# jliu/graph-normalizing-flows

Measured on AMD Instinct MI355X. Metric: node-updates/sec (fwd+logdet) on community_medium batch, higher is better.
Workload: dtype f32; 1 GPU; config2: community_medium batch=64/GPU (64 graphs total), 8-step GRevNet fwd+logdet, D=64 L=256 K=5 avg_then_mlp eps=1 leaky_relu(0.2), sparse topology+self loops; nodes_total=2718, edges_total=32202, nodes_rank0=2718, edges_rank0=32202, weights=N(0,2/(fan_in+fan_out)), seed 99, last layer x0.25, parallelism=single GPU

## Files before the change

graph-normalizing-flows_amd/csrc/gnf_fused.hip:

```cpp
#include <cstring>
#include "gnf_common.h"

namespace gnf {

static constexpr int kFusedThreads = 512;
static constexpr int kLdsLimit = 160 * 1024;
static constexpr int kRowptrPad = 40;
static constexpr int kColCap = 2048;

static inline int pad16(int v) { return (v + 15) & ~15; }

int64_t packed_floats(const GnfMlp* m) {
    int64_t tot = 0;
    for (int j = 0; j < m->num_layers; ++j) {
        const int64_t ip = pad16(m->dims[j]), op = pad16(m->dims[j + 1]);
        tot += 2 * ip * op + op;
    }
    return tot;
}

__global__ __launch_bounds__(256) void k_pack_layer(const float* __restrict__ W,
                                                    const float* __restrict__ b, int I, int O, int Ip,
                                                    int Op, float* __restrict__ wout,
                                                    float* __restrict__ bout, float* __restrict__ wtout) {
    const int64_t nw = (int64_t)Ip * Op;
    const int64_t i = (int64_t)blockIdx.x * 256 + threadIdx.x;
    if (i < nw) {
        const int q = (int)(i & 3);
        const int lane = (int)((i >> 2) & 63);
        const int64_t blk = i >> 8;
        const int kgs = Ip >> 4;
        const int nts = Op >> 4;
        const int kg = (int)(blk / nts), nt = (int)(blk % nts);
        (void)kgs;
        const int k = 16 * kg + 4 * (lane >> 4) + q;
        const int c = 16 * nt + (lane & 15);
        wout[i] = (k < I && c < O) ? W[(int64_t)k * O + c] : 0.f;
        const int nts_t = Ip >> 4;
        const int kg_t = (int)(blk / nts_t), nt_t = (int)(blk % nts_t);
        const int ko = 16 * kg_t + 4 * (lane >> 4) + q;
        const int ci = 16 * nt_t + (lane & 15);
        wtout[i] = (ci < I && ko < O) ? W[(int64_t)ci * O + ko] : 0.f;
    } else if (i < nw + Op) {
        const int c = (int)(i - nw);
        bout[c] = c < O ? b[c] : 0.f;
    }
}

static int64_t packed_weight_floats(const GnfMlp* m) {
    int64_t tot = 0;
    for (int j = 0; j < m->num_layers; ++j) tot += (int64_t)pad16(m->dims[j]) * pad16(m->dims[j + 1]);
    return tot;
}

int launch_pack_mlp(const GnfMlp* m, float* packed, hipStream_t st) {
    int64_t woff = 0, boff = packed_weight_floats(m);
    int64_t toff = boff;
    for (int j = 0; j < m->num_layers; ++j) toff += pad16(m->dims[j + 1]);
    for (int j = 0; j < m->num_layers; ++j) {
        const int I = m->dims[j], O = m->dims[j + 1], Ip = pad16(I), Op = pad16(O);
        const int64_t tot = (int64_t)Ip * Op + Op;
        hipLaunchKernelGGL(k_pack_layer, dim3((unsigned)((tot + 255) / 256)), dim3(256), 0, st, m->W[j],
                           m->b[j], I, O, Ip, Op, packed + woff, packed + boff, packed + toff + woff);
        GNF_LAUNCH_CHECK("k_pack_layer");
        woff += (int64_t)Ip * Op;
        boff += Op;
    }
    return GNF_OK;
}


}
#include "gnf_fused_dev.h"
#include "gnf_attn_front_dev.h"
namespace gnf {

#ifdef GNF_TRACE
static constexpr int kTraceSlots = 32, kTraceCoupled = kTraceSlots - 2, kTraceEnd = kTraceSlots - 1;
static constexpr int kTracePhFlushed = 20;
__shared__ unsigned long long s_trace[kFusedThreads / 64][kTraceSlots];
static unsigned long long* g_trace_buf = nullptr;
static int g_trace_cap = 0, g_trace_next = 0;
extern "C" __attribute__((visibility("default"))) void gnf_trace_set_buffer(unsigned long long* buf, int cap) {
    g_trace_buf = buf, g_trace_cap = cap, g_trace_next = 0;
}
__device__ __forceinline__ void geo_stamp(int slot) {
    __builtin_amdgcn_sched_barrier(0);
    const unsigned long long t = __builtin_readcyclecounter();
    if ((threadIdx.x & 63) == 0) s_trace[threadIdx.x >> 6][slot] = t;
    __builtin_amdgcn_sched_barrier(0);
}
__device__ __forceinline__ void geo_stamp_after(int slot, float landed) {
    asm volatile("" ::"v"(landed));
    geo_stamp(slot);
}
#define GNF_STAMP(SLOT) geo_stamp(SLOT)
#define GNF_STAMP_AFTER(SLOT, V) geo_stamp_after(SLOT, V)
#else
#define GNF_STAMP(SLOT) ((void)0)
#define GNF_STAMP_AFTER(SLOT, V) ((void)0)
#endif

template <class Mv>
__device__ __forceinline__ double add_moved(double v, Mv&& mv) {
    const int lo = mv(__double2loint(v)), hi = mv(__double2hiint(v));
    return v + __hiloint2double(hi, lo);
}
__device__ __forceinline__ double wave_sum_lane0(double v) {
    v = add_moved(v, [](int x) { return (int)__builtin_amdgcn_permlane32_swap((unsigned)x, (unsigned)x, false, false)[1]; });
    v = add_moved(v, [](int x) { return (int)__builtin_amdgcn_permlane16_swap((unsigned)x, (unsigned)x, false, false)[1]; });
    v = add_moved(v, [](int x) { return __builtin_amdgcn_update_dpp(0, x, 0x108, 0xf, 0xf, true); });
    v = add_moved(v, [](int x) { return __builtin_amdgcn_update_dpp(0, x, 0x104, 0xf, 0xf, true); });
    v = add_moved(v, [](int x) { return __builtin_amdgcn_update_dpp(0, x, 0x102, 0xf, 0xf, true); });
    v = add_moved(v, [](int x) { return __builtin_amdgcn_update_dpp(0, x, 0x101, 0xf, 0xf, true); });
    return v;
}

struct CoupleOwn {
    float xu = 0.f;
    float* dst = nullptr;
    double* part = nullptr;
    double* sq_part = nullptr;
    int inverse = 0;
};
template <int TM, bool STASH, bool FRONT, bool ROWLD, bool PLAIN, class Args, class FArgs, class RArgs>
__device__ __forceinline__ void couple_tile(const Args& a, const FArgs& fa, const RArgs& rla, const int H, const int LS, float* s_lds,
                                            const float* t_lds, float* xn_lds, const float* bn_lds, double* red, int tile, int row0,
                                            int tid, int wave, int lane, [[maybe_unused]] const CoupleOwn& own = CoupleOwn{}) {
    [[maybe_unused]] auto bn_part = [&]() -> double* {
        if constexpr (PLAIN) return nullptr; else return a.bn_part;
    };
    double local = 0.0, local2 = 0.0;
    for (int idx = tid; idx < TM * H; idx += kFusedThreads) {
        const int rl = idx / H, f = idx - rl * H;
        const int r = row0 + rl;
        if (bn_part()) xn_lds[rl * LS + f] = 0.f;
        bool live;
        if constexpr (PLAIN) live = own.dst != nullptr; else live = r < a.n_nodes;
        if (live) {
            float sv = s_lds[rl * LS + f], tv = t_lds[rl * LS + f];
            [[maybe_unused]] const int HPb = (H + 15) & ~15;
            if constexpr (!PLAIN) {
                if (a.residual) {
                    float xr = a.x_cond[(int64_t)r * a.ld + f];
                    if constexpr (FRONT) {
                        if (fa.bn_part) xr = xr * bn_lds[f] + bn_lds[HPb + f];
                    }
                    sv += xr;
                    tv += xr;
                }
            }
            float xv;
            if constexpr (PLAIN) xv = own.xu; else xv = a.x_upd_src[(int64_t)r * a.ld + f];
            if constexpr (FRONT) {
                if (a.bnu_const) xv = xv * bn_lds[2 * HPb + f] + bn_lds[3 * HPb + f];
                else if (a.bnu_inv[0]) xv = (xv - bn_lds[f]) / bn_lds[HPb + f] * bn_lds[2 * HPb + f] + bn_lds[3 * HPb + f];
            }
            int inverse;
            if constexpr (PLAIN) inverse = own.inverse; else inverse = a.inverse;
            const float xn = inverse ? (xv - tv) * expf(-sv) : xv * expf(sv) + tv;
            if constexpr (PLAIN) *own.dst = xn; else a.x_upd[(int64_t)r * a.ld + f] = xn;
            local += (double)sv;
            local2 += (double)xn * (double)xn;
            if constexpr (ROWLD) s_lds[rl * LS + f] = sv;
            if (bn_part()) xn_lds[rl * LS + f] = xn;
            if constexpr (STASH) {
                a.stash_st[0][(int64_t)r * H + f] = sv;
                a.stash_st[1][(int64_t)r * H + f] = tv;
            }
        }
    }
    if constexpr (PLAIN) GNF_STAMP(kTraceCoupled);
    if constexpr (PLAIN) {
        constexpr int NW = kFusedThreads / 64;
        const bool sq = own.sq_part != nullptr;
        local = wave_sum_lane0(local);
        if (sq) local2 = wave_sum_lane0(local2);
        if (lane == 0) {
            red[wave] = local;
            if (sq) red[NW + wave] = local2;
        }
        __syncthreads();
        if (tid == 0) {
            double tot = 0.0 + local;
            for (int w = 1; w < NW; ++w) tot += red[w];
            *own.part = tot;
            if (sq) {
                double tot2 = 0.0 + local2;
                for (int w = 1; w < NW; ++w) tot2 += red[NW + w];
                *own.sq_part = tot2;
            }
        }
        return;
    }
    for (int off = 32; off > 0; off >>= 1) local += __shfl_down(local, off, 64);
    if (lane == 0) red[wave] = local;
    __syncthreads();
    if (tid == 0) {
        double tot = 0.0;
        for (int w = 0; w < kFusedThreads / 64; ++w) tot += red[w];
        a.partials[tile] = tot;
    }
    if constexpr (!PLAIN) {
        if (a.bn_part) {
            __syncthreads();
            for (int i = tid; i < 2 * H; i += kFusedThreads) {
                const int f = i >> 1, which = i & 1;
                double acc = 0.0;
                for (int rl = 0; rl < TM; ++rl) {
                    const double v = (double)xn_lds[rl * LS + f];
                    acc += which ? v * v : v;
                }
                a.bn_part[((int64_t)tile * H + f) * 2 + which] = acc;
            }
        }
    }
    if (a.sq_partials) {
        for (int off = 32; off > 0; off >>= 1) local2 += __shfl_down(local2, off, 64);
        __syncthreads();
        if (lane == 0) red[wave] = local2;
        __syncthreads();
        if (tid == 0) {
            double tot = 0.0;
            for (int w = 0; w < kFusedThreads / 64; ++w) tot += red[w];
            a.sq_partials[tile] = tot;
        }
    }
    if constexpr (ROWLD) {
        __syncthreads();
        constexpr int TPR = kFusedThreads / TM;
        const int rl = tid / TPR, l = tid % TPR;
        double acc = 0.0;
        for (int f = l; f < H; f += TPR) acc += (double)s_lds[rl * LS + f];
        for (int off = TPR / 2; off > 0; off >>= 1) acc += __shfl_down(acc, off, TPR);
        if (l == 0 && row0 + rl < a.n_nodes) rla.row[row0 + rl] = acc;
    }
}

__device__ __forceinline__ int nets2_tile(int bid, int nwg) {
    const int xcd = bid & 7, qd = nwg >> 3, rm = nwg & 7;
    return (xcd < rm ? xcd * (qd + 1) : rm * (qd + 1) + (xcd - rm) * qd) + (bid >> 3);
}

template <int MT, int NETS, bool STASH = false, bool FRONT = false, bool FIXED = false, bool ROWLD = false>
__global__ __launch_bounds__(kFusedThreads) void k_half_fused(const FusedArgs a, const FrontArgs fa, const RowLdArgs rla) {
    extern __shared__ __attribute__((aligned(16))) float smem[];
    static_assert(!FRONT || (MT == 1 && NETS == 2), "the attention prologue exists for the 16-row both-nets shape");
    static_assert(!ROWLD || (NETS == 2 && !STASH), "per-row log-det: the both-nets inference instances (one net per workgroup couples in k_coupling)");
    constexpr int TM = 16 * MT;
    constexpr int WPN = 8 / NETS;
    const int LS = a.LS;
    auto buf = [&](int net_, int pp_) -> float* { return smem + (2 * net_ + pp_) * TM * LS; };
    int base_floats = 2 * NETS * TM * LS;
    if constexpr (FRONT) {
// ... 182 lines not shown
        const bool v4 = (a.in0 & 3) == 0 && ((reinterpret_cast<uintptr_t>(a.h0[net0]) | reinterpret_cast<uintptr_t>(a.h0[NETS == 2 ? 1 : net0])) & 15) == 0;
        if (v4) {
            const int q4 = in0p >> 2;
            for (int idx = tid; idx < TM * q4; idx += kFusedThreads) {
                const int rl = idx / q4, c = (idx - rl * q4) * 4;
                const int r = row0 + rl;
                const bool live = r < a.n_nodes && c < a.in0;
                const f32x4 z4 = {0.f, 0.f, 0.f, 0.f};
                const f32x4 v0 = live ? *reinterpret_cast<const f32x4*>(a.h0[net0] + (int64_t)r * a.in0 + c) : z4;
                f32x4 v1 = z4;
                if (NETS == 2 && live) v1 = *reinterpret_cast<const f32x4*>(a.h0[1] + (int64_t)r * a.in0 + c);
                *reinterpret_cast<f32x4*>(buf(0, 0) + rl * LS + c) = v0;
                if (NETS == 2) *reinterpret_cast<f32x4*>(buf(1, 0) + rl * LS + c) = v1;
            }
        } else
        for (int idx = tid; idx < TM * in0p; idx += kFusedThreads) {
            const int rl = idx / in0p, c = idx - rl * in0p;
            const int r = row0 + rl;
            const bool live = r < a.n_nodes && c < a.in0;
            buf(0, 0)[rl * LS + c] = live ? a.h0[net0][(int64_t)r * a.in0 + c] : 0.f;
            if (NETS == 2) buf(1, 0)[rl * LS + c] = live ? a.h0[1][(int64_t)r * a.in0 + c] : 0.f;
        }
    } else {
        const TileAgg ta{a.col, a.x_cond, a.ld, a.n_nodes, row0, H, a.in0, a.ipg[0] * 16, a.mean, a.concat, a.eps, a.cond_copy};
        tile_aggregate<TM, kFusedThreads, kColCap>(ta, s_rowptr, s_col, buf(0, 0), NETS == 2 ? buf(1, 0) : nullptr, LS,
                                                   STASH ? a.stash_h0 : nullptr, tid);
    }
    __syncthreads();
    }

    int pp = 0;
    for (int j = 0; j < a.K; ++j) {
        const float* in_lds = buf(nl, pp);
        float* out_lds = buf(nl, pp ^ 1);
        const float slope = (j == a.K - 1) ? 1.f : (a.act == GNF_ACT_RELU ? 0.f : a.alpha);
        while (cur.layer == j) {
            const WChunk c = cur;
            const WChunk nxt = next_chunk(c);
            const WChunk nx = nxt.layer < a.K ? nxt : c;
            const float* bl = bias_lds + nl * a.bias_tot + c.boff;
            constexpr bool kThin = MT == 1;
            const bool thin_ok = kThin && thin_for(j), thin_nx = kThin && thin_for(nx.layer);
            constexpr int EPI = STASH ? EPI_EX : EPI_PLAIN;
            EpiArgs ea{};
            if constexpr (STASH) {
                ea.mode = 0;
                ea.mask = j < a.K - 1 ? fmask + (size_t)(nl * (a.K - 1) + j) * (MT * 4) * a.stash_mld : nullptr;
                ea.mld = a.stash_mld;
            }
            if (c.nv >= 4)
                mlp_chunk<MT, 4, EPI>(in_lds, LS, c, nx, WPN, bl, out_lds, slope, lane, b_pre, ea, thin_nx);
            else if (c.nv == 3)
                mlp_chunk<MT, 3, EPI>(in_lds, LS, c, nx, WPN, bl, out_lds, slope, lane, b_pre, ea, thin_nx);
            else if (c.nv == 2)
                mlp_chunk<MT, 2, EPI>(in_lds, LS, c, nx, WPN, bl, out_lds, slope, lane, b_pre, ea, thin_nx);
            else if (kThin && thin_ok && chunk_is_thin(c))
                mlp_chunk_thin(in_lds, LS, c, nx, WPN, bl, out_lds, slope, lane, b_pre);
            else
                mlp_chunk<MT, 1, EPI>(in_lds, LS, c, nx, WPN, bl, out_lds, slope, lane, b_pre, ea, thin_nx);
            cur = nxt;
        }
        if constexpr (STASH && NETS == 2) {
            if (j >= 1) {
#pragma unroll
                for (int q = 0; q < 2; ++q)
                    tile_dump<TM, kFusedThreads, true>(buf(q, pp), LS, a.stash_act[q][j], (int64_t)a.stash_ld, a.stash_w[j - 1], row0,
                                                       a.n_nodes, tid);
            }
        }
        pp ^= 1;
        __syncthreads();
    }

    if constexpr (STASH) {
        const int total_words = 2 * (a.K - 1) * (MT * 4) * a.stash_mld;
        unsigned long long* gm = a.stash_mask + (size_t)tile * total_words;
        for (int i = tid; i < total_words; i += kFusedThreads) gm[i] = fmask[i];
    }
    if (NETS == 1) {
        const float* o_lds = buf(0, pp);
        float* dst = a.st_out[net0];
        for (int idx = tid; idx < TM * H; idx += kFusedThreads) {
            const int rl = idx / H, f = idx - rl * H;
            const int r = row0 + rl;
            if (r < a.n_nodes)
                dst[(int64_t)r * H + f] = o_lds[rl * LS + f] + (a.residual ? a.x_cond[(int64_t)r * a.ld + f] : 0.f);
        }
    } else {
        couple_tile<TM, STASH, FRONT, ROWLD, false>(a, fa, rla, H, LS, buf(0, pp), buf(1, pp), buf(0, pp ^ 1), bn_lds, red, tile, row0, tid,
                                                    wave, lane);
    }
}


struct GeoArgs {
    const int32_t* rowptr;
    const int32_t* col;
    const float* x_cond;
    float* x_upd;
    const float* x_upd_src;
    float* cond_copy;
    double* partials;
    double* sq_partials;
    const float* wp[2];
    int64_t ld;
    int32_t n_nodes, n_tiles;
    float eps, alpha;
    int32_t mean, act, inverse;
#ifdef GNF_TRACE
    unsigned long long* trace;
#endif
};

template <class T>
__device__ __forceinline__ T hold_v(T v) {
    asm volatile("" : "+v"(v));
    return v;
}
template <class T>
__device__ __forceinline__ T* hold_v(T* p) {
    asm volatile("" : "+v"(p));
    return (T*)(__attribute__((address_space(1))) T*)p;
}

template <int IN0G, int LG, int K, int HG>
struct GeoLayout {
    static constexpr int kWpn = 4;
    static constexpr int kFragFloats = 64 * 4;
    static_assert(kFragFloats * sizeof(float) == 1024 && sizeof(f32x4) == 16, "GNF_LOAD_B addresses 1 KiB fragment blocks, 16 bytes per lane");
    static_assert(K >= 2 && IN0G >= 1 && IN0G == HG, "combine = agg: the layer-0 input is as wide as the half that is rewritten");
    static_assert(LG == 4 * kWpn, "a wave owns exactly four column tiles of a hidden layer: one mlp_chunk<1, 4> per layer");
    static_assert(HG <= kWpn && LG <= kThinStages, "the output layer is at most one thin chunk per wave");
    static constexpr int ipg(int j) { return j == 0 ? IN0G : LG; }
    static constexpr int ont(int j) { return j == K - 1 ? HG : LG; }
    static constexpr int woff(int j) { return j == 0 ? 0 : woff(j - 1) + ipg(j - 1) * ont(j - 1) * kFragFloats; }
    static constexpr int boff(int j) { return j == 0 ? 0 : boff(j - 1) + 16 * ont(j - 1); }
    static constexpr int kBias = woff(K);
    static constexpr int kLS = 16 * (LG > IN0G ? LG : IN0G) + 4;
    static constexpr int kRed = 2 * (kFusedThreads / 64);
    static constexpr int kBiasBlock = boff(K);
    static constexpr size_t kBiasAt = (size_t)2 * 2 * 16 * kLS * sizeof(float) + kRed * sizeof(double) + (kRowptrPad + kColCap) * sizeof(int);
    static constexpr size_t kLds = kBiasAt + (size_t)2 * kBiasBlock * sizeof(float);
    static_assert(kBiasAt % 16 == 0 && kBiasBlock % 4 == 0, "the bias block is written and read in 16-byte pieces");
    static_assert(2 * (kBiasBlock / 4) <= 2 * kFusedThreads && 2 * (kBiasBlock / 4) - kFusedThreads <= 16,
                  "one 16-byte piece per thread, and a second one for at most 16 threads");
    static_assert(kLds > (size_t)kLdsLimit / 2, "one workgroup per CU");
    static_assert(woff(1) == 16 * IN0G * 16 * LG && kBias == 16 * IN0G * 16 * LG + (K - 2) * 256 * LG * LG + 16 * LG * 16 * HG,
                  "sum of Ip x Op over the layers");
    static_assert(kLds <= (size_t)kLdsLimit, "activation buffers in LDS");
    static_assert(LG == 2 * kPhaseTs && kPhaseTs == kFusedThreads / 64, "a wave owns exactly two column tiles of a hidden layer of EACH net: one mlp_phase per net and layer");
    static_assert(2 * HG <= kWpn, "the output layer's 2 HG accumulator chains go to waves 0 .. 2 HG - 1: one per SIMD");
};

template <int IN0G, int LG, int K, int HG, bool PHASES = false>
__global__ __launch_bounds__(kFusedThreads) void k_half_fused_geo(const GeoArgs a) {
    extern __shared__ __attribute__((aligned(16))) float smem[];
    using G = GeoLayout<IN0G, LG, K, HG>;
    constexpr int TM = 16, WPN = G::kWpn, LS = G::kLS, H = 16 * HG, IN0 = 16 * IN0G;
    static_assert(TM * H == kFusedThreads && IN0 == H, "one own-row element per thread, the same one in the gather and in the coupling");
    GNF_STAMP(0);
    auto buf = [&](int net_, int pp_) -> float* { return smem + (2 * net_ + pp_) * TM * LS; };
    double* red = reinterpret_cast<double*>(smem + 2 * 2 * TM * LS);
    int* s_rowptr = reinterpret_cast<int*>(red + G::kRed);
    int* s_col = s_rowptr + kRowptrPad;
    [[maybe_unused]] float* s_bias = smem + G::kBiasAt / sizeof(float);

    const int tid = threadIdx.x;
    const int wave = __builtin_amdgcn_readfirstlane(tid >> 6), lane = tid & 63;
    const int nl = wave / WPN;
    const int wl = (wave % WPN + nl * (WPN / 2)) % WPN;
    const int voff = lane * 16;

    const float* wnet = a.wp[PHASES ? 0 : nl];
    [[maybe_unused]] const float* wnet1 = a.wp[1];
    [[maybe_unused]] const int wt_own = (wave + kPhaseTs - HG) % kPhaseTs;
    if constexpr (PHASES) asm volatile("" ::"s"(wnet1));
#ifdef GNF_TRACE
    asm volatile("" ::"s"(a.trace));
#endif
    asm volatile("" ::"s"(a.rowptr), "s"(a.col), "s"(a.x_cond), "s"(a.x_upd), "s"(a.x_upd_src), "s"(a.cond_copy), "s"(a.partials),
                 "s"(a.sq_partials), "s"(wnet), "s"(a.ld), "s"(a.n_nodes), "s"(a.n_tiles), "s"(a.eps), "s"(a.alpha), "s"(a.mean), "s"(a.act),
                 "s"(a.inverse));
    const int tile = nets2_tile(blockIdx.x, a.n_tiles);
    const int row0 = tile * TM;

    const int rp_row = row0 + (lane < TM ? lane : TM);
    const int rp_reg = a.rowptr[rp_row < a.n_nodes ? rp_row : a.n_nodes];
    CoupleOwn own;
    float xc_own;
    {
        const int r = row0 + tid / H, f = tid % H;
        const bool live = r < a.n_nodes;
        const int64_t at = (int64_t)(live ? r : a.n_nodes - 1) * a.ld + f;
        xc_own = a.x_cond[at];
        own.xu = a.x_upd_src[at];
        own.dst = hold_v(live ? a.x_upd + at : nullptr);
        own.part = hold_v(a.partials + tile);
        own.sq_part = hold_v(a.sq_partials ? a.sq_partials + tile : nullptr);
        own.inverse = hold_v(a.inverse);
    }
    [[maybe_unused]] constexpr int NPC = G::kBiasBlock / 4;
    [[maybe_unused]] f32x4 bias_pc, bias_pc2;
    [[maybe_unused]] const int bias_at2 = kFusedThreads + (lane & 15);
    static_assert(kFusedThreads >= NPC && kFusedThreads + 15 < 2 * NPC, "pieces past kFusedThreads are the second net's");
    if constexpr (PHASES) {
        bias_pc = *reinterpret_cast<const f32x4*>((tid < NPC ? wnet : wnet1) + G::kBias + 4 * (tid < NPC ? tid : tid - NPC));
        bias_pc2 = *reinterpret_cast<const f32x4*>(wnet1 + G::kBias + 4 * (bias_at2 - NPC));
    }
    __builtin_amdgcn_sched_barrier(0);

    auto chunk = [&](auto jc) -> WChunk {
        constexpr int j = decltype(jc)::value;
        WChunk c;
        c.wbase = wnet + G::woff(j);
        c.wbytes = (unsigned)G::ipg(j) * (unsigned)G::ont(j) * 1024u;
        c.ipg = G::ipg(j);
        c.ont = G::ont(j);
        c.boff = G::boff(j);
        c.nt0 = wl;
        c.nv = j == K - 1 ? 1 : 4;
        c.layer = j;
        return c;
    };
    const bool last_mine = wl < HG;

    if (tid <= TM) s_rowptr[tid] = rp_reg;
    const int seg_beg = __builtin_amdgcn_readlane(rp_reg, 0);
    const int seg_len = __builtin_amdgcn_readlane(rp_reg, TM) - seg_beg;
    GNF_STAMP(1);

    const bool staged = seg_len <= kColCap;
    int col_reg = 0;
    if (staged && tid < seg_len) col_reg = a.col[seg_beg + tid];
    __builtin_amdgcn_sched_barrier(0);
    f32x4 b_pre[kPF][4];
    [[maybe_unused]] f32x4 ph_b_pre[kPhasePF][2];
    [[maybe_unused]] auto ph_pf = [](int j) constexpr { return G::ipg(j) < kPhasePF ? G::ipg(j) : kPhasePF; };
    [[maybe_unused]] f32x4 ph_bias[2][K - 1][2];
    [[maybe_unused]] const int thin_net = wave >= HG && wave < 2 * HG;
    [[maybe_unused]] const bool thin_mine = wave < 2 * HG;
    [[maybe_unused]] const int thin_tile = thin_mine ? (thin_net ? wt_own : wave) : 0;
    BiasRegs<4> bias_h[K - 1];
    BiasRegs<1> bias_o;
    if constexpr (PHASES) {
        const __amdgpu_buffer_rsrc_t rs0 =
            __builtin_amdgcn_make_buffer_rsrc(const_cast<float*>(wnet), 0, G::ipg(0) * G::ont(0) * 1024, 0x00020000);
#pragma unroll
        for (int u = 0; u < ph_pf(0); ++u)
#pragma unroll
            for (int b = 0; b < 2; ++b) ph_b_pre[u][b] = GNF_LOAD_B(rs0, voff, (u * G::ont(0) + wave + kPhaseTs * b) * 1024);
    } else {
    prefetch_chunk(chunk(std::integral_constant<int, 0>{}), WPN, voff, b_pre, true);
    const float* bnet = wnet + G::kBias + 16 * wl + (lane & 15);
#pragma unroll
    for (int j = 0; j < K - 1; ++j)
#pragma unroll
        for (int b = 0; b < 4; ++b) bias_h[j].v[b] = bnet[G::boff(j) + 16 * WPN * b];
    bias_o.v[0] = bnet[G::boff(K - 1) - (last_mine ? 0 : 16 * wl)];
    }
    __builtin_amdgcn_sched_barrier(0);
    if constexpr (PHASES) {
        *reinterpret_cast<f32x4*>(s_bias + 4 * tid) = bias_pc;
        if (tid < 2 * NPC - kFusedThreads) *reinterpret_cast<f32x4*>(s_bias + 4 * bias_at2) = bias_pc2;
    }
    if (staged) {
        if (tid < seg_len) s_col[tid] = col_reg;
        for (int i = tid + kFusedThreads; i < seg_len; i += kFusedThreads) s_col[i] = a.col[seg_beg + i];
    }
    __syncthreads();
    GNF_STAMP(2);
    if constexpr (PHASES) {
        __builtin_amdgcn_sched_barrier(0);
#pragma unroll
        for (int q = 0; q < 2; ++q) {
            const float* bq = s_bias + q * G::kBiasBlock + 16 * (q ? wt_own : wave) + 4 * (lane >> 4);
#pragma unroll
            for (int j = 0; j < K - 1; ++j)
#pragma unroll
                for (int b = 0; b < 2; ++b) ph_bias[q][j][b] = *reinterpret_cast<const f32x4*>(bq + G::boff(j) + 16 * kPhaseTs * b);
        }
        bias_o.v[0] = s_bias[thin_net * G::kBiasBlock + G::boff(K - 1) + 16 * thin_tile + (lane & 15)];
    }
    const TileAgg ta{a.col, a.x_cond, a.ld, a.n_nodes, row0, H, IN0, IN0, a.mean, 0, a.eps, a.cond_copy};
    tile_gather<TM, kFusedThreads, kColCap>(ta, s_rowptr, s_col, buf(0, 0), buf(1, 0), LS, nullptr, tid, OwnRow{xc_own});
    __syncthreads();
    GNF_STAMP(3);

    const float slope_h = a.act == GNF_ACT_RELU ? 0.f : a.alpha;
    if constexpr (PHASES) {
        const int lrow = lane & 15, lgrp = lane >> 4;
        const int lane_at = lrow * LS + 4 * lgrp;
        f32x4 acc_s[2], acc_t[2], a_pre[kPhasePF];
#pragma unroll
        for (int u = 0; u < ph_pf(0); ++u) a_pre[u] = *reinterpret_cast<const f32x4*>(buf(0, 0) + lane_at + 16 * u);
        WChunk thin;
        thin.wbase = (thin_net ? wnet1 : wnet) + G::woff(K - 1);
        thin.wbytes = (unsigned)G::ipg(K - 1) * (unsigned)G::ont(K - 1) * 1024u;
        thin.ipg = G::ipg(K - 1), thin.ont = G::ont(K - 1), thin.boff = G::boff(K - 1), thin.nt0 = thin_tile, thin.nv = 1, thin.layer = K - 1;
        epi_static_for<K - 1>([&](auto jc) {
            constexpr int j = decltype(jc)::value;
            constexpr int pj = j & 1;
#pragma unroll
            for (int b = 0; b < 2; ++b) acc_s[b] = ph_bias[0][j][b];
            GNF_STAMP(4 + 4 * j);
            mlp_phase<G::ipg(j), G::ont(j), ph_pf(j), (j > 0), PH_NEXT_HIDDEN, G::ipg(j), G::ont(j), ph_pf(j)>(
                buf(0, pj) + lane_at, wnet + G::woff(j), wave, acc_s, a_pre, ph_b_pre, acc_t, buf(1, pj) + lane_at + 16 * wt_own, slope_h,
                buf(1, pj) + lane_at, wnet1 + G::woff(j), wt_own, thin, b_pre, voff, [&] { GNF_STAMP(5 + 4 * j); });
#pragma unroll
            for (int b = 0; b < 2; ++b) acc_t[b] = ph_bias[1][j][b];
            GNF_STAMP(6 + 4 * j);
            constexpr int jn = j + 1 < K - 1 ? j + 1 : j;
            mlp_phase<G::ipg(j), G::ont(j), ph_pf(j), true, (j + 1 < K - 1 ? PH_NEXT_HIDDEN : PH_NEXT_THIN), G::ipg(jn), G::ont(jn), ph_pf(jn)>(
                buf(1, pj) + lane_at, wnet1 + G::woff(j), wt_own, acc_t, a_pre, ph_b_pre, acc_s, buf(0, pj ^ 1) + lane_at + 16 * wave, slope_h,
                buf(0, pj ^ 1) + lane_at, wnet + G::woff(jn), wave, thin, b_pre, voff, [&] { GNF_STAMP(7 + 4 * j); });
        });
        constexpr int po = (K - 1) & 1;
        phase_flush(acc_t, buf(1, po) + lane_at + 16 * wt_own, slope_h);
        GNF_STAMP(kTracePhFlushed);
        phase_barrier();
        GNF_STAMP(kTracePhFlushed + 1);
        if (thin_mine) mlp_chunk_thin(buf(thin_net, po), LS, thin, thin, kPhaseTs, bias_o, buf(thin_net, po ^ 1), 1.f, lane, b_pre);
        __syncthreads();
        GNF_STAMP(kTracePhFlushed + 2);
    } else
    epi_static_for<K>([&](auto jc) {
        constexpr int j = decltype(jc)::value;
        const float* in_lds = buf(nl, j & 1);
        float* out_lds = buf(nl, (j & 1) ^ 1);
        const WChunk c = chunk(jc);
        GNF_STAMP_AFTER(4 + 2 * j, b_pre[0][0][0]);
        if constexpr (j < K - 2) {
            mlp_chunk<1, 4>(in_lds, LS, c, chunk(std::integral_constant<int, j + 1>{}), WPN, bias_h[j], out_lds, slope_h, lane, b_pre, EpiArgs{}, true);
        } else if constexpr (j == K - 2) {
            const WChunk nx = last_mine ? chunk(std::integral_constant<int, K - 1>{}) : c;
            mlp_chunk<1, 4>(in_lds, LS, c, nx, WPN, bias_h[j], out_lds, slope_h, lane, b_pre, EpiArgs{}, true);
        } else {
            if (last_mine) mlp_chunk_thin(in_lds, LS, c, c, WPN, bias_o, out_lds, 1.f, lane, b_pre);
        }
        __syncthreads();
        GNF_STAMP(5 + 2 * j);
    });

    constexpr int pp = K & 1;
    couple_tile<TM, false, false, false, true>(a, 0, 0, H, LS, buf(0, pp), buf(1, pp), buf(0, pp ^ 1), nullptr, red, tile, row0, tid, wave, lane, own);
    GNF_STAMP(kTraceEnd);
#ifdef GNF_TRACE
    static_assert(4 + 2 * K <= kTraceCoupled && 4 + 4 * (K - 1) <= kTracePhFlushed, "stamp slots");
    if (a.trace && (blockIdx.x == 0 || blockIdx.x == gridDim.x / 2) && lane < kTraceSlots)
        a.trace[((blockIdx.x != 0) * (kFusedThreads / 64) + wave) * kTraceSlots + lane] = s_trace[wave][lane];
#endif
}

static int max_padded_width(const GnfMlp* m) {
    int w = 16;
    for (int j = 0; j <= m->num_layers; ++j) w = w > pad16(m->dims[j]) ? w : pad16(m->dims[j]);
    return w;
}

static int bias_total(const GnfMlp* m) {
    int t = 0;
    for (int j = 0; j < m->num_layers; ++j) t += pad16(m->dims[j + 1]);
    return t;
}

static size_t fused_lds_bytes(const GnfMlp* m, int MT, int NETS) {
    const int LS = max_padded_width(m) + 4;
    return (size_t)(2 * NETS * 16 * MT * LS + NETS * bias_total(m) + 2) * sizeof(float) + 8 * sizeof(double) +
           (GNF_MAX_LAYERS * 8 + kRowptrPad + kColCap) * sizeof(int);
}

bool fused_fits_lds(const GnfMlp* m) { return fused_lds_bytes(m, 1, 1) <= (size_t)kLdsLimit; }

static void choose_shape(const HalfStep& hs, int* mt, int* nets);
static int choose_big(const HalfStep& hs);

bool fused_supported(const HalfStep& hs) {
    const GnfMlp *s = hs.s_net, *t = hs.t_net;
    if (!s->packed || !t->packed) return false;
    if (s->num_layers != t->num_layers) return false;
    for (int j = 0; j <= s->num_layers; ++j)
        if (s->dims[j] != t->dims[j]) return false;
    return fused_lds_bytes(s, 1, 1) <= (size_t)kLdsLimit;
}

bool fused_supports_oop(const HalfStep& hs) {
    if (!fused_supported(hs) || hs.s_net->attn) return false;
    if (choose_big(hs)) return true;
    int mt, nets;
    choose_shape(hs, &mt, &nets);
    return nets == 2;
}

static void choose_shape(const HalfStep& hs, int* mt, int* nets) {
    const GnfMlp* s = hs.s_net;
    const int64_t tiles16 = (hs.n_nodes + 15) / 16;
    auto fits = [&](int m, int n) { return fused_lds_bytes(s, m, n) <= (size_t)kLdsLimit; };
    int m = 1, n = 1;
    const int64_t cus = big_cu_count();
    if (tiles16 > cus && fits(2, 2)) {
        m = 2, n = 2;
    } else if (fits(1, 2)) {
        m = 1, n = 2;
    } else if (tiles16 > cus && fits(2, 1)) {
        m = 2, n = 1;
    }
    if (const int64_t force = opt(OPT_FORCE_SHAPE)) {
        const int fm = (int)(force / 10), fn = (int)(force % 10);
        if ((fm == 1 || fm == 2) && (fn == 1 || fn == 2) && fits(fm, fn)) m = fm, n = fn;
    }
    if (s->attn && s->attn->layer_norm) n = 1;
    *mt = m;
    *nets = n;
}

static int choose_big(const HalfStep& hs) {
    const GnfMlp* s = hs.s_net;
    if (!big_supported(s, hs.H) || hs.mlp_stash) return 0;
    if (hs.n_nodes * hs.ld >= (int64_t(1) << 31)) return 0;
    if (s->attn && s->attn->layer_norm) return 0;
    if (const int64_t force = opt(OPT_FORCE_SHAPE)) {
        if (force == kForceBigLostPartner) return 4;
        return (force % 10 == 0 && force >= 10 && force <= 40) ? (int)(force / 10) : 0;
    }
    const int64_t g = (hs.n_nodes + 15) / 16, c = big_cu_count();
    if (g <= 2 * c) return 0;
    const double old_q = (double)((g + 2 * c - 1) / (2 * c));
    double big_q;
    if (g <= 8 * c) {
        big_q = 1.22 + 0.525 * (double)g / (double)(2 * c);
    } else {
        static const double closing[8] = {0.0, 0.8, 1.25, 1.7, 2.18, 2.4, 2.6, 3.0};
        const int64_t full = g / (8 * c), left = g - full * 8 * c, t = (left + c - 1) / c;
        big_q = 3.36 * (double)full + 0.15 + (t <= 7 ? closing[t] : 3.36);
    }
    return big_q < old_q ? 4 : 0;
}

// ... 307 lines not shown
```

Measured before the change: 47.24 million node-updates/s.

## Gather CSR neighbours per wave via scalar loads in the phased kernel

In the PHASES path, each wave now owns two rows. It reads their rowptr and column indices through scalar constant-address loads instead of staging the column list in LDS. It then issues the neighbour feature loads directly, with up to 24 edges per row held in registers, before the barrier, and finishes the sum and writes both activation buffers afterwards. The layer-0 weight prefetch can be placed before, between or after the gather requests through a macro; the default issues it after the column fetch. This removes the LDS staging of column indices and one barrier dependency, and overlaps the gather latency with the bias store. The cost is more register pressure and a serial fallback loop for rows of high degree.

```diff
diff --git a/graph-normalizing-flows_amd/csrc/gnf_fused.hip b/graph-normalizing-flows_amd/csrc/gnf_fused.hip
--- a/graph-normalizing-flows_amd/csrc/gnf_fused.hip
+++ b/graph-normalizing-flows_amd/csrc/gnf_fused.hip
@@ -78,6 +78,7 @@
 #ifdef GNF_TRACE
 static constexpr int kTraceSlots = 32, kTraceCoupled = kTraceSlots - 2, kTraceEnd = kTraceSlots - 1;
 static constexpr int kTracePhFlushed = 20;
+static constexpr int kTraceCsrIssued = 23;
 __shared__ unsigned long long s_trace[kFusedThreads / 64][kTraceSlots];
 static unsigned long long* g_trace_buf = nullptr;
 static int g_trace_cap = 0, g_trace_next = 0;
@@ -100,6 +101,10 @@
 #define GNF_STAMP(SLOT) ((void)0)
 #define GNF_STAMP_AFTER(SLOT, V) ((void)0)
 #endif
+
+}
+#include "gnf_fused_geo_csr_dev.h"
+namespace gnf {
 
 template <class Mv>
 __device__ __forceinline__ double add_moved(double v, Mv&& mv) {
@@ -588,6 +593,10 @@
     static_assert(2 * HG <= kWpn, "the output layer's 2 HG accumulator chains go to waves 0 .. 2 HG - 1: one per SIMD");
 };
 
+#ifndef GNF_GEO_WEIGHTS_AT
+#define GNF_GEO_WEIGHTS_AT 1
+#endif
+static constexpr int kGeoWeightsAt = GNF_GEO_WEIGHTS_AT;
 template <int IN0G, int LG, int K, int HG, bool PHASES = false>
 __global__ __launch_bounds__(kFusedThreads) void k_half_fused_geo(const GeoArgs a) {
     extern __shared__ __attribute__((aligned(16))) float smem[];
@@ -620,8 +629,15 @@
     const int tile = nets2_tile(blockIdx.x, a.n_tiles);
     const int row0 = tile * TM;
 
-    const int rp_row = row0 + (lane < TM ? lane : TM);
-    const int rp_reg = a.rowptr[rp_row < a.n_nodes ? rp_row : a.n_nodes];
+    [[maybe_unused]] GeoCsrRows csr;
+    [[maybe_unused]] int rp_reg = 0;
+    if constexpr (PHASES) {
+        csr = geo_csr_rowptr(a.rowptr, row0 + 2 * wave, a.n_nodes);
+        __builtin_amdgcn_sched_barrier(0);
+    } else {
+        const int rp_row = row0 + (lane < TM ? lane : TM);
+        rp_reg = a.rowptr[rp_row < a.n_nodes ? rp_row : a.n_nodes];
+    }
     CoupleOwn own;
     float xc_own;
     {
@@ -643,6 +659,17 @@
         bias_pc = *reinterpret_cast<const f32x4*>((tid < NPC ? wnet : wnet1) + G::kBias + 4 * (tid < NPC ? tid : tid - NPC));
         bias_pc2 = *reinterpret_cast<const f32x4*>(wnet1 + G::kBias + 4 * (bias_at2 - NPC));
     }
+    [[maybe_unused]] f32x4 ph_b_pre[kPhasePF][2];
+    [[maybe_unused]] auto ph_pf = [](int j) constexpr { return G::ipg(j) < kPhasePF ? G::ipg(j) : kPhasePF; };
+    [[maybe_unused]] auto load_s0_weights = [&] {
+        const __amdgpu_buffer_rsrc_t rs0 =
+            __builtin_amdgcn_make_buffer_rsrc(const_cast<float*>(wnet), 0, G::ipg(0) * G::ont(0) * 1024, 0x00020000);
+#pragma unroll
+        for (int u = 0; u < ph_pf(0); ++u)
+#pragma unroll
+            for (int b = 0; b < 2; ++b) ph_b_pre[u][b] = GNF_LOAD_B(rs0, voff, (u * G::ont(0) + wave + kPhaseTs * b) * 1024);
+    };
+    if constexpr (PHASES && kGeoWeightsAt == 0) load_s0_weights();
     __builtin_amdgcn_sched_barrier(0);
 
     auto chunk = [&](auto jc) -> WChunk {
@@ -660,31 +687,38 @@
     };
     const bool last_mine = wl < HG;
 
-    if (tid <= TM) s_rowptr[tid] = rp_reg;
-    const int seg_beg = __builtin_amdgcn_readlane(rp_reg, 0);
-    const int seg_len = __builtin_amdgcn_readlane(rp_reg, TM) - seg_beg;
-    GNF_STAMP(1);
-
-    const bool staged = seg_len <= kColCap;
-    int col_reg = 0;
-    if (staged && tid < seg_len) col_reg = a.col[seg_beg + tid];
+    [[maybe_unused]] int seg_beg = 0, seg_len = 0;
+    if constexpr (!PHASES) {
+        if (tid <= TM) s_rowptr[tid] = rp_reg;
+        seg_beg = __builtin_amdgcn_readlane(rp_reg, 0);
+        seg_len = __builtin_amdgcn_readlane(rp_reg, TM) - seg_beg;
+        GNF_STAMP(1);
+    }
+
+    [[maybe_unused]] const bool staged = seg_len <= kColCap;
+    [[maybe_unused]] int col_reg = 0;
+    if constexpr (!PHASES) {
+        if (staged && tid < seg_len) col_reg = a.col[seg_beg + tid];
+    }
     __builtin_amdgcn_sched_barrier(0);
     f32x4 b_pre[kPF][4];
-    [[maybe_unused]] f32x4 ph_b_pre[kPhasePF][2];
-    [[maybe_unused]] auto ph_pf = [](int j) constexpr { return G::ipg(j) < kPhasePF ? G::ipg(j) : kPhasePF; };
     [[maybe_unused]] f32x4 ph_bias[2][K - 1][2];
     [[maybe_unused]] const int thin_net = wave >= HG && wave < 2 * HG;
     [[maybe_unused]] const bool thin_mine = wave < 2 * HG;
     [[maybe_unused]] const int thin_tile = thin_mine ? (thin_net ? wt_own : wave) : 0;
     BiasRegs<4> bias_h[K - 1];
     BiasRegs<1> bias_o;
+    [[maybe_unused]] GeoCsrGather csr_g;
+    [[maybe_unused]] const bool csr_hi = lane >= H;
     if constexpr (PHASES) {
-        const __amdgpu_buffer_rsrc_t rs0 =
-            __builtin_amdgcn_make_buffer_rsrc(const_cast<float*>(wnet), 0, G::ipg(0) * G::ont(0) * 1024, 0x00020000);
-#pragma unroll
-        for (int u = 0; u < ph_pf(0); ++u)
-#pragma unroll
-            for (int b = 0; b < 2; ++b) ph_b_pre[u][b] = GNF_LOAD_B(rs0, voff, (u * G::ont(0) + wave + kPhaseTs * b) * 1024);
+        const GeoCsrCols csr_c = geo_csr_cols(csr, a.col);
+        asm volatile("" ::"v"(bias_pc), "v"(bias_pc2));
+        *reinterpret_cast<f32x4*>(s_bias + 4 * tid) = bias_pc;
+        if (tid < 2 * NPC - kFusedThreads) *reinterpret_cast<f32x4*>(s_bias + 4 * bias_at2) = bias_pc2;
+        __builtin_amdgcn_sched_barrier(0);
+        if constexpr (kGeoWeightsAt == 1) load_s0_weights();
+        csr_g = geo_csr_request(csr, csr_c, a.x_cond + tid % H, a.ld, csr_hi);
+        if constexpr (kGeoWeightsAt == 2) load_s0_weights();
     } else {
     prefetch_chunk(chunk(std::integral_constant<int, 0>{}), WPN, voff, b_pre, true);
     const float* bnet = wnet + G::kBias + 16 * wl + (lane & 15);
@@ -695,16 +729,14 @@
     bias_o.v[0] = bnet[G::boff(K - 1) - (last_mine ? 0 : 16 * wl)];
     }
     __builtin_amdgcn_sched_barrier(0);
-    if constexpr (PHASES) {
-        *reinterpret_cast<f32x4*>(s_bias + 4 * tid) = bias_pc;
-        if (tid < 2 * NPC - kFusedThreads) *reinterpret_cast<f32x4*>(s_bias + 4 * bias_at2) = bias_pc2;
-    }
-    if (staged) {
-        if (tid < seg_len) s_col[tid] = col_reg;
-        for (int i = tid + kFusedThreads; i < seg_len; i += kFusedThreads) s_col[i] = a.col[seg_beg + i];
+    if constexpr (!PHASES) {
+        if (staged) {
+            if (tid < seg_len) s_col[tid] = col_reg;
+            for (int i = tid + kFusedThreads; i < seg_len; i += kFusedThreads) s_col[i] = a.col[seg_beg + i];
+        }
     }
     __syncthreads();
-    GNF_STAMP(2);
+    if constexpr (!PHASES) GNF_STAMP(2);
     if constexpr (PHASES) {
         __builtin_amdgcn_sched_barrier(0);
 #pragma unroll
@@ -717,8 +749,17 @@
         }
         bias_o.v[0] = s_bias[thin_net * G::kBiasBlock + G::boff(K - 1) + 16 * thin_tile + (lane & 15)];
     }
-    const TileAgg ta{a.col, a.x_cond, a.ld, a.n_nodes, row0, H, IN0, IN0, a.mean, 0, a.eps, a.cond_copy};
-    tile_gather<TM, kFusedThreads, kColCap>(ta, s_rowptr, s_col, buf(0, 0), buf(1, 0), LS, nullptr, tid, OwnRow{xc_own});
+    if constexpr (PHASES) {
+        __builtin_amdgcn_sched_barrier(0);
+        const int rl = tid / H, f = tid % H;
+        const bool live = row0 + rl < a.n_nodes;
+        float* cond_dst = a.cond_copy && live ? a.cond_copy + (int64_t)(row0 + rl) * a.ld + f : nullptr;
+        geo_csr_finish(csr_g, csr, a.col, a.x_cond + f, a.ld, csr_hi, live, xc_own, cond_dst, a.mean, a.eps, buf(0, 0) + rl * LS + f,
+                       buf(1, 0) + rl * LS + f);
+    } else {
+        const TileAgg ta{a.col, a.x_cond, a.ld, a.n_nodes, row0, H, IN0, IN0, a.mean, 0, a.eps, a.cond_copy};
+        tile_gather<TM, kFusedThreads, kColCap>(ta, s_rowptr, s_col, buf(0, 0), buf(1, 0), LS, nullptr, tid, OwnRow{xc_own});
+    }
     __syncthreads();
     GNF_STAMP(3);
 
diff --git a/graph-normalizing-flows_amd/csrc/gnf_fused_geo_csr_dev.h b/graph-normalizing-flows_amd/csrc/gnf_fused_geo_csr_dev.h
--- /dev/null
+++ b/graph-normalizing-flows_amd/csrc/gnf_fused_geo_csr_dev.h
@@ -0,0 +1,163 @@
+#pragma once
+#include "gnf_fused_dev.h"
+
+namespace gnf {
+
+#define GNF_CSR_CONST __attribute__((address_space(4)))
+typedef int csr_i32x8 __attribute__((ext_vector_type(8)));
+typedef csr_i32x8 csr_i32x8_dw __attribute__((aligned(4)));
+
+static constexpr int kCsrChunks = 3;
+
+struct GeoCsrRows {
+    int beg[2], end[2], n_edges;
+};
+
+struct GeoCsrCols {
+    csr_i32x8 a[kCsrChunks], b[kCsrChunks];
+};
+
+struct GeoCsrGather {
+    float vv[8 * kCsrChunks];
+    int deg;
+    int n_up;
+};
+
+__device__ __forceinline__ GeoCsrRows geo_csr_rowptr(const int32_t* rowptr, int row_a, int n_nodes) {
+    const GNF_CSR_CONST int32_t* rp = (const GNF_CSR_CONST int32_t*)rowptr;
+    const int r0 = row_a < n_nodes ? row_a : n_nodes, r1 = row_a + 1 < n_nodes ? row_a + 1 : n_nodes,
+              r2 = row_a + 2 < n_nodes ? row_a + 2 : n_nodes;
+    GeoCsrRows c;
+    c.beg[0] = rp[r0];
+    c.end[0] = c.beg[1] = rp[r1];
+    c.end[1] = rp[r2];
+    c.n_edges = rp[n_nodes];
+    return c;
+}
+
+__device__ __forceinline__ csr_i32x8 geo_csr_chunk(const GNF_CSR_CONST int32_t* col, int want, int end, int n_edges) {
+    csr_i32x8 c = {0, 0, 0, 0, 0, 0, 0, 0};
+    if (want < end) {
+        if (want + 8 <= n_edges) {
+            c = *reinterpret_cast<const GNF_CSR_CONST csr_i32x8_dw*>(col + want);
+        } else {
+#pragma unroll
+            for (int q = 0; q < 8; ++q) c[q] = col[want + q < n_edges ? want + q : n_edges - 1];
+        }
+    }
+    return c;
+}
+
+__device__ __forceinline__ void geo_csr_move_down(csr_i32x8& c, int shift) {
+#pragma unroll
+    for (int b = 4; b; b >>= 1)
+        if (shift & b) {
+#pragma unroll
+            for (int q = 0; q + b < 8; ++q) c[q] = c[q + b];
+        }
+}
+
+template <bool LD32>
+__device__ __forceinline__ void geo_csr_rows(const csr_i32x8& ca, const csr_i32x8& cb, bool hi, const float* xf, int64_t ld,
+                                             uint32_t ld_bytes, float* vv) {
+#pragma unroll
+    for (int q = 0; q < 8; ++q) {
+        const int ci = hi ? cb[q] : ca[q];
+        if constexpr (LD32)
+            vv[q] = *reinterpret_cast<const float*>(reinterpret_cast<const char*>(xf) + (uint64_t)(uint32_t)ci * ld_bytes);
+        else
+            vv[q] = xf[(int64_t)ci * ld];
+    }
+}
+__device__ __forceinline__ bool geo_csr_ld32(int64_t ld) { return (uint64_t)ld < (1ull << 30); }
+
+__device__ __forceinline__ GeoCsrCols geo_csr_cols(const GeoCsrRows& c, const int32_t* col_) {
+    const GNF_CSR_CONST int32_t* col = (const GNF_CSR_CONST int32_t*)col_;
+#ifdef GNF_TRACE
+    asm volatile("" ::"s"(c.beg[0]), "s"(c.end[0]), "s"(c.end[1]), "s"(c.n_edges));
+    GNF_STAMP(1);
+#endif
+    GeoCsrCols cc;
+    csr_i32x8 (&ca)[kCsrChunks] = cc.a, (&cb)[kCsrChunks] = cc.b;
+    if (c.n_edges >= 8) {
+        int sa[kCsrChunks], sb[kCsrChunks], any = 0;
+#pragma unroll
+        for (int k = 0; k < kCsrChunks; ++k) {
+            const int wa = c.beg[0] + 8 * k, wb = c.beg[1] + 8 * k, last = c.n_edges - 8;
+            const int fa = wa < last ? wa : last, fb = wb < last ? wb : last;
+            sa[k] = wa - fa, sb[k] = wb - fb, any |= sa[k] | sb[k];
+            ca[k] = *reinterpret_cast<const GNF_CSR_CONST csr_i32x8_dw*>(col + fa);
+            cb[k] = *reinterpret_cast<const GNF_CSR_CONST csr_i32x8_dw*>(col + fb);
+        }
+        if (any) {
+#pragma unroll
+            for (int k = 0; k < kCsrChunks; ++k) geo_csr_move_down(ca[k], sa[k]), geo_csr_move_down(cb[k], sb[k]);
+        }
+    } else {
+#pragma unroll
+        for (int k = 0; k < kCsrChunks; ++k) {
+            ca[k] = geo_csr_chunk(col, c.beg[0] + 8 * k, c.end[0], c.n_edges);
+            cb[k] = geo_csr_chunk(col, c.beg[1] + 8 * k, c.end[1], c.n_edges);
+        }
+    }
+    return cc;
+}
+
+__device__ __forceinline__ GeoCsrGather geo_csr_request(const GeoCsrRows& c, const GeoCsrCols& cc, const float* xf, int64_t ld, bool hi) {
+    const csr_i32x8 (&ca)[kCsrChunks] = cc.a, (&cb)[kCsrChunks] = cc.b;
+    const int deg_a = c.end[0] - c.beg[0], deg_b = c.end[1] - c.beg[1];
+    const int deg_max = deg_a > deg_b ? deg_a : deg_b;
+    GeoCsrGather g;
+    g.deg = hi ? deg_b : deg_a;
+    g.n_up = geo_csr_ld32(ld) ? (deg_max < 8 * kCsrChunks ? deg_max : 8 * kCsrChunks) : 0;
+    const uint32_t ld_bytes = (uint32_t)__builtin_amdgcn_readfirstlane((int)((uint32_t)ld * 4u));
+#ifdef GNF_TRACE
+    asm volatile("" ::"s"(ca[kCsrChunks - 1][7]), "s"(cb[kCsrChunks - 1][7]));
+    GNF_STAMP(2);
+#endif
+#pragma unroll
+    for (int k = 0; k < kCsrChunks; ++k)
+        if (8 * k < g.n_up) geo_csr_rows<true>(ca[k], cb[k], hi, xf, ld, ld_bytes, g.vv + 8 * k);
+    __builtin_amdgcn_sched_barrier(0);
+    GNF_STAMP(kTraceCsrIssued);
+    return g;
+}
+
+__device__ __forceinline__ void geo_csr_finish(const GeoCsrGather& g, const GeoCsrRows& c, const int32_t* col_, const float* xf, int64_t ld,
+                                               bool hi, bool live, float xc, float* cond_dst, int mean, float eps, float* out0, float* out1) {
+    const GNF_CSR_CONST int32_t* col = (const GNF_CSR_CONST int32_t*)col_;
+    float s = 0.f;
+    asm volatile("" : "+v"(s));
+#pragma unroll
+    for (int k = 0; k < kCsrChunks; ++k)
+        if (8 * k < g.n_up) {
+#pragma unroll
+            for (int q = 0; q < 8; ++q)
+                if (8 * k + q < g.deg) s += g.vv[8 * k + q];
+        }
+#ifdef GNF_TRACE
+    asm volatile("" ::"v"(s));
+    GNF_STAMP(kTraceCsrIssued + 1);
+#endif
+    const int deg_a = c.end[0] - c.beg[0], deg_b = c.end[1] - c.beg[1];
+    const int deg_max = deg_a > deg_b ? deg_a : deg_b;
+    for (int base = g.n_up ? 8 * kCsrChunks : 0; base < deg_max; base += 8) {
+        const csr_i32x8 ca = geo_csr_chunk(col, c.beg[0] + base, c.end[0], c.n_edges);
+        const csr_i32x8 cb = geo_csr_chunk(col, c.beg[1] + base, c.end[1], c.n_edges);
+        float vv[8];
+        geo_csr_rows<false>(ca, cb, hi, xf, ld, 0u, vv);
+#pragma unroll
+        for (int q = 0; q < 8; ++q)
+            if (base + q < g.deg) s += vv[q];
+    }
+    if (mean) s = s / (float)(g.deg > 1 ? g.deg : 1);
+    float v = 0.f;
+    if (live) {
+        if (cond_dst) *cond_dst = xc;
+        v = eps * xc + s;
+    }
+    *out0 = v;
+    *out1 = v;
+}
+
+}
```

Result: faster. 47.84 million node-updates/s, median of 6 (+1.3%).
